# YuxinxinChen/dlrm-yx

Hardware: AMD Instinct MI355X
Metric: DLRM samples/sec fwd+bwd at 1/2/4/8 MI355X; embedding HBM GB/s vs peak (higher is better)
Workload: dtype fp32; 1 GPU; mlperf_terabyte_synthetic; global_batch=2048, local_batch=2048, tables=26, rows_total=54063992, emb_dim=128, lookups_per_bag=1, optimizer=sgd, parallelism=table-sharded emb x1 + dp1, hip_graph=True, capture=whole, bot_sched=auto, tbe_role=True, bottom_parts=0, head_role=True, early_sort=True, feature_pad=False

## Files before the change

dlrm-yx_amd/csrc/gemm.hip:

```cpp
#include <cstdlib>
#include <cstring>
#include <type_traits>

#include "common.hpp"
#include "tbe_bwd_roles.hpp"

#ifndef DLRM_GEMM_STAMP
#define DLRM_GEMM_STAMP(slot)
#endif

namespace {

using f32x16 = __attribute__((ext_vector_type(16))) float;
using f32x4 = __attribute__((ext_vector_type(4))) float;
constexpr int kThreads = 256;
constexpr int kMaxSplit = 32;
constexpr int kMaxGroup = 6;
constexpr int64_t kTicketCap = 16384;
constexpr int kBK = 32;
constexpr int kRasterRows = 4;

struct GemmParams {
  int64_t M, N, K;
  float alpha;
  const float* A;
  int64_t lda;
  const float* B;
  int64_t ldb;
  float* C;
  int64_t ldc;
  int epi;
  const float* bias;
  const float* aux;
  int64_t ldaux;
  int64_t ones_col;
  int layout;
  int tiles_m, tiles_n;
  int splits;
  int block0;
  int64_t kchunk;
  float* ws;
  int* counters;
  int mode;
  float* part;
  const float* alpha_dev;
};

struct GemmGroup {
  GemmParams p[kMaxGroup];
  int n;
  int total;
};

__device__ __forceinline__ int swz_kc(int r) {
  return ((r >> 1) & 7) ^ (((unsigned)((r & 15) - 4) < 8u) ? 2 : 0);
}

template <int MN, int BKT, bool KC, bool VEC, int NT, bool SWZ = false>
struct Stage {
  static_assert(!SWZ || (BKT % 32 == 0 && MN >= 32), "swizzled images: BKT 32 U, MN >= 32");
  static constexpr int PITCH = SWZ ? (KC ? 32 : MN) : (KC ? BKT + 4 : MN + 4);
  static constexpr int SIZE = SWZ ? MN * BKT : (KC ? MN * PITCH : BKT * PITCH);
  __device__ __forceinline__ static int at(int mn, int k) {
    if constexpr (!SWZ) return KC ? mn * PITCH + k : k * PITCH + mn;
    else if constexpr (KC)
      return ((k >> 5) * MN + mn) * 32 + 4 * (((k & 31) >> 2) ^ swz_kc(mn)) + (k & 3);
    else return k * PITCH + (mn ^ (((k >> 3) & 1) << 4));
  }
  static constexpr int NV = MN * BKT / 4 / NT;
  static_assert(NV >= 1 && MN * BKT % (4 * NT) == 0, "panel / thread mismatch");
  float4 regs[NV];

  __device__ __forceinline__ void coords(int q, int& mn, int& k) const {
    if constexpr (KC && SWZ) {
      const int u = q / (MN * 8), r = q - u * (MN * 8);
      mn = r >> 3;
      k = 32 * u + 4 * (r & 7);
    } else if constexpr (KC) {
      mn = q / (BKT / 4);
      k = 4 * (q % (BKT / 4));
    } else {
      k = q / (MN / 4);
      mn = 4 * (q % (MN / 4));
    }
  }

  __device__ __forceinline__ void load(const float* __restrict__ X, int64_t ld, int64_t mn0,
                                       int64_t mnlim, int64_t k0, int64_t klim, int tid) {
    if (VEC && mn0 + MN <= mnlim && k0 + BKT <= klim) {
#pragma unroll
      for (int v = 0; v < NV; ++v) {
        int mn, k;
        coords(tid + v * NT, mn, k);
        const float* ptr = KC ? X + (mn0 + mn) * ld + k0 + k : X + (k0 + k) * ld + mn0 + mn;
        regs[v] = *reinterpret_cast<const float4*>(ptr);
      }
      return;
    }
#pragma unroll
    for (int v = 0; v < NV; ++v) {
      int mn, k;
      coords(tid + v * NT, mn, k);
      const int64_t gmn = mn0 + mn, gk = k0 + k;
      const float* ptr = KC ? X + gmn * ld + gk : X + gk * ld + gmn;
      const bool full = KC ? (gmn < mnlim && gk + 3 < klim) : (gk < klim && gmn + 3 < mnlim);
      if (VEC && full) {
        regs[v] = *reinterpret_cast<const float4*>(ptr);
      } else {
        float e[4];
#pragma unroll
        for (int c = 0; c < 4; ++c) {
          const bool ok = KC ? (gmn < mnlim && gk + c < klim) : (gk < klim && gmn + c < mnlim);
          e[c] = ok ? ptr[c] : 0.f;
        }
        regs[v] = make_float4(e[0], e[1], e[2], e[3]);
      }
    }
  }

  __device__ __forceinline__ void load_one(int v, const float* __restrict__ X, int64_t ld,
                                           int64_t mn0, int64_t mnlim, int64_t k0, int64_t klim,
                                           int tid, bool fast) {
    int mn, k;
    coords(tid + v * NT, mn, k);
    const int64_t gmn = mn0 + mn, gk = k0 + k;
    const float* ptr = KC ? X + gmn * ld + gk : X + gk * ld + gmn;
    if (VEC && fast) {
      regs[v] = *reinterpret_cast<const float4*>(ptr);
      return;
    }
    float e[4];
#pragma unroll
    for (int c = 0; c < 4; ++c) {
      const bool ok = KC ? (gmn < mnlim && gk + c < klim) : (gk < klim && gmn + c < mnlim);
      e[c] = ok ? ptr[c] : 0.f;
    }
    regs[v] = make_float4(e[0], e[1], e[2], e[3]);
  }

  __device__ __forceinline__ void load_one4(int v, __amdgpu_buffer_rsrc_t rsrc, int64_t ld,
                                            int64_t mn0, int64_t mnlim, int64_t k0, int64_t klim,
                                            int tid) {
    int mn, k;
    coords(tid + v * NT, mn, k);
    const int64_t gmn = mn0 + mn, gk = k0 + k;
    const bool ok = gmn < mnlim && gk < klim;
    const int64_t e = KC ? gmn * ld + gk : gk * ld + gmn;
    const int off = ok ? (int)(e * 4) : 0x7ffffff0;
    const auto t = __builtin_amdgcn_raw_buffer_load_b128(rsrc, off, 0, 0);
    regs[v] = __builtin_bit_cast(float4, t);
  }

  struct Fetch {
    int off[NV];
    int kpos[NV];
  };
  __device__ __forceinline__ void fetch_init(Fetch& f, int64_t ld, int64_t mn0, int64_t mnlim,
                                             int64_t kbeg, int tid) const {
#pragma unroll
    for (int v = 0; v < NV; ++v) {
      int mn, k;
      coords(tid + v * NT, mn, k);
      const int64_t gmn = mn0 + mn, gk = kbeg + k;
      const int64_t e = KC ? gmn * ld + gk : gk * ld + gmn;
      f.off[v] = (KC || gmn < mnlim) ? (int)(e * 4) : -1;
      f.kpos[v] = k;
    }
  }
  __device__ __forceinline__ void fetch4(int v, const Fetch& f, __amdgpu_buffer_rsrc_t rsrc,
                                         int tile_step, int t, int kt0, int klim) {
    const bool ok = f.off[v] >= 0 && kt0 + f.kpos[v] < klim;
    const int off = ok ? f.off[v] + t * tile_step : 0x7ffffff0;
    regs[v] = __builtin_bit_cast(float4, __builtin_amdgcn_raw_buffer_load_b128(rsrc, off, 0, 0));
  }

  __device__ __forceinline__ void fetch4s(int v, const Fetch& f, __amdgpu_buffer_rsrc_t rsrc,
                                          int soff) {
    const int off = f.off[v] >= 0 ? f.off[v] : 0x7ffffff0;
    regs[v] = __builtin_bit_cast(float4, __builtin_amdgcn_raw_buffer_load_b128(rsrc, off, soff, 0));
  }

  __device__ __forceinline__ void store_one(int v, float* __restrict__ lds, int tid) const {
    int mn, k;
    coords(tid + v * NT, mn, k);
    *reinterpret_cast<float4*>(lds + at(mn, k)) = regs[v];
  }

  __device__ __forceinline__ void store(float* __restrict__ lds, int tid) const {
#pragma unroll
    for (int v = 0; v < NV; ++v) store_one(v, lds, tid);
  }

  template <int NS>
  __device__ __forceinline__ void frag(const float* __restrict__ lds, int off, int l32, int kbase,
                                       float (&f)[NS]) const {
    static_assert(NS % 4 == 0, "fragment length");
    if constexpr (KC) {
#pragma unroll
      for (int c = 0; c < NS / 4; ++c) {
        const float4 v = *reinterpret_cast<const float4*>(lds + at(off + l32, kbase + 4 * c));
        f[4 * c + 0] = v.x;
        f[4 * c + 1] = v.y;
        f[4 * c + 2] = v.z;
        f[4 * c + 3] = v.w;
      }
    } else {
#pragma unroll
      for (int s = 0; s < NS; ++s) f[s] = lds[at(off + l32, kbase + s)];
    }
  }
};

__device__ __forceinline__ float add_f32(float a, float b) {
// ... 158 lines not shown
                                            rr, (o + tid * NV + 4 * q) * 4, 0, 16));
#pragma unroll
    for (int i = 0; i < FM; ++i)
      tr[i] = __builtin_bit_cast(float, __builtin_amdgcn_raw_buffer_load_b32(
                                            rr, (o + BM * BN + rrow + i * rs_stride) * 4, 0, 16));
  };
  auto add_rec = [&](const float4 (&t)[NV / 4], const float (&tr)[FM], bool first) {
#pragma unroll
    for (int q = 0; q < NV / 4; ++q) {
      v[4 * q + 0] = first ? t[q].x : v[4 * q + 0] + t[q].x;
      v[4 * q + 1] = first ? t[q].y : v[4 * q + 1] + t[q].y;
      v[4 * q + 2] = first ? t[q].z : v[4 * q + 2] + t[q].z;
      v[4 * q + 3] = first ? t[q].w : v[4 * q + 3] + t[q].w;
    }
#pragma unroll
    for (int i = 0; i < FM; ++i) rs[i] = first ? tr[i] : rs[i] + tr[i];
  };
  int s = 0;
  for (; s + 1 < p.splits; s += 2) {
    float4 t0[NV / 4], t1[NV / 4];
    float r0[FM], r1[FM];
    load_rec(s, t0, r0);
    load_rec(s + 1, t1, r1);
    add_rec(t0, r0, s == 0);
    add_rec(t1, r1, false);
  }
  if (s < p.splits) {
    float4 t0[NV / 4];
    float r0[FM];
    load_rec(s, t0, r0);
    add_rec(t0, r0, s == 0);
  }
  return true;
}

template <int BM, int BN, int WGM, int WGN, bool RS, int FM, int FN>
__device__ __forceinline__ void finish_tile(const GemmParams& p, float alpha,
                                            const f32x4 (&acc)[FM][FN], float (&rs)[FM], int tile,
                                            int split, int tn, int64_t m0, int64_t n0,
                                            float* smem) {
  constexpr int WM = BM / WGM, WN = BN / WGN;
  const int tid = threadIdx.x;
  const int wave = tid >> 6;
  const int lane = tid & 63;
  const int kq = lane >> 4;
  const int l16 = lane & 15;
  const int wm0 = (wave / WGN) * WM;
  const int wn0 = (wave % WGN) * WN;
  const bool rs_owner = RS && tn == 0 && (wave % WGN) == 0 && kq == 0;

  constexpr int NV = FM * FN * 4;
  float v[NV];
#pragma unroll
  for (int i = 0; i < FM; ++i)
#pragma unroll
    for (int j = 0; j < FN; ++j)
#pragma unroll
      for (int r = 0; r < 4; ++r) v[(i * FN + j) * 4 + r] = acc[i][j][r];
  if (p.mode == DLRM_GEMM_PARTIAL) {
    float* slab = p.part + (int64_t)split * p.M * p.N;
    if (p.M * p.N * 4 < 0x7ff00000LL) {
      const __amdgpu_buffer_rsrc_t rp = __builtin_amdgcn_make_buffer_rsrc(
          (void*)slab, (short)0, (int)(p.M * p.N * 4), 0x00020000);
#pragma unroll
      for (int i = 0; i < FM; ++i)
#pragma unroll
        for (int j = 0; j < FN; ++j) {
          const int col = (int)(n0 + wn0 + j * 16 + l16);
#pragma unroll
          for (int r = 0; r < 4; ++r) {
            const int row = (int)(m0 + wm0 + i * 16 + 4 * kq + r);
            buf_st(v[(i * FN + j) * 4 + r], rp,
                   row < p.M && col < p.N ? (int)(((int64_t)row * p.N + col) * 4) : kOob);
          }
        }
    } else {
#pragma unroll
      for (int i = 0; i < FM; ++i)
#pragma unroll
        for (int j = 0; j < FN; ++j) {
          const int64_t col = n0 + wn0 + j * 16 + l16;
#pragma unroll
          for (int r = 0; r < 4; ++r) {
            const int64_t row = m0 + wm0 + i * 16 + 4 * kq + r;
            if (row < p.M && col < p.N) slab[row * p.N + col] = v[(i * FN + j) * 4 + r];
          }
        }
    }
    if (rs_owner) {
      float* rslab = p.part + (int64_t)p.splits * p.M * p.N + (int64_t)split * p.M;
#pragma unroll
      for (int i = 0; i < FM; ++i) {
        const int64_t row = m0 + wm0 + i * 16 + l16;
        if (row < p.M) rslab[row] = rs[i];
      }
    }
    return;
  }
  if (!splitk_reduce<BM, BN, NV, FM>(p, tile, split, v, rs, wm0 + l16, 16, rs_owner, smem))
    return;
  if (epi_fits(p)) {
    int row[NV], col[NV];
    bool ok[NV];
    float w[NV];
#pragma unroll
    for (int i = 0; i < FM; ++i)
#pragma unroll
      for (int j = 0; j < FN; ++j)
#pragma unroll
        for (int r = 0; r < 4; ++r) {
          const int q = (i * FN + j) * 4 + r;
          row[q] = (int)(m0 + wm0 + i * 16 + 4 * kq + r);
          col[q] = (int)(n0 + wn0 + j * 16 + l16);
          ok[q] = col[q] < p.N;
          w[q] = dlrm_scale(alpha, v[q]);
        }
    store_elems_any<NV>(p, row, col, ok, w);
    if constexpr (RS) {
      int rrow[FM], rcol[FM];
      bool rok[FM];
      float rw[FM];
#pragma unroll
      for (int i = 0; i < FM; ++i) {
        rrow[i] = (int)(m0 + wm0 + i * 16 + l16);
        rcol[i] = (int)p.ones_col;
        rok[i] = rs_owner;
        rw[i] = dlrm_scale(alpha, rs[i]);
      }
      store_elems_any<FM>(p, rrow, rcol, rok, rw);
    }
    return;
  }
#pragma unroll
  for (int i = 0; i < FM; ++i)
#pragma unroll
    for (int j = 0; j < FN; ++j) {
      const int64_t col = n0 + wn0 + j * 16 + l16;
#pragma unroll
      for (int r = 0; r < 4; ++r) {
        const int64_t row = m0 + wm0 + i * 16 + 4 * kq + r;
        if (row < p.M && col < p.N) store_epilogue(p, row, col, alpha, v[(i * FN + j) * 4 + r]);
      }
    }
  if (rs_owner) {
#pragma unroll
    for (int i = 0; i < FM; ++i) {
      const int64_t row = m0 + wm0 + i * 16 + l16;
      if (row < p.M) store_epilogue(p, row, p.ones_col, alpha, rs[i]);
    }
  }
}


template <int BM, int BN, int WGM, int WGN, bool A_KC, bool B_KC, bool RS, int U = 1>
__device__ __forceinline__ void pipe_body(const GemmParams& p, int lb, float* smem) {
  static_assert(U == 1 || U % 2 == 0, "sub-tiles per stage: 1 or even");
  constexpr int NT = WGM * WGN * 64;
  constexpr int WM = BM / WGM, WN = BN / WGN;
  constexpr int FM = WM / 16, FN = WN / 16;
  static_assert(FM >= 1 && FN >= 1, "wave sub-tile");
  constexpr int KL = kBK / 4;
  constexpr int BKT = kBK * U;
  using SA = Stage<BM, BKT, A_KC, true, NT, true>;
  using SB = Stage<BN, BKT, B_KC, true, NT, true>;
  constexpr int NS = SA::NV + SB::NV;
  static_assert(NS <= U * KL - 1, "staging must finish before the barrier step");

  const float alpha = dlrm_resolve_lr(p.alpha_dev, p.alpha);
  const int tile = lb / p.splits;
  const int split = lb - tile * p.splits;
  int tm, tn;
  {
    constexpr int G = kRasterRows;
    const int per_group = G * p.tiles_n;
    const int grp = tile / per_group, first = grp * G;
    const int gsz = p.tiles_m - first < G ? p.tiles_m - first : G;
    const int pos = tile - grp * per_group;
    tm = first + pos % gsz;
    tn = pos / gsz;
  }
  if constexpr (RS) {
    if (tn != 0) return pipe_body<BM, BN, WGM, WGN, A_KC, B_KC, false, U>(p, lb, smem);
  }
  const int64_t m0 = (int64_t)tm * BM;
  const int64_t n0 = (int64_t)tn * BN;
  const int64_t kbeg = (int64_t)split * p.kchunk;
  const int64_t kend = (kbeg + p.kchunk < p.K) ? kbeg + p.kchunk : p.K;

  const int tid = threadIdx.x;
  const int wave = tid >> 6;
  const int lane = tid & 63;
  const int kq = lane >> 4;
  const int l16 = lane & 15;
  const int wm0 = (wave / WGN) * WM;
  const int wn0 = (wave % WGN) * WN;

  f32x4 acc[FM][FN];
#pragma unroll
  for (int i = 0; i < FM; ++i)
#pragma unroll
    for (int j = 0; j < FN; ++j) acc[i][j] = f32x4{0.f, 0.f, 0.f, 0.f};
  float rs[FM];
#pragma unroll
  for (int i = 0; i < FM; ++i) rs[i] = 0.f;

  const int nsub = (int)((kend - kbeg + kBK - 1) / kBK);
  const int nk = (nsub + U - 1) / U;
  SA sa;
  SB sb;
  const int64_t a_ext = A_KC ? (p.M - 1) * p.lda + p.K : (p.K - 1) * p.lda + p.M;
  const int64_t b_ext = B_KC ? (p.N - 1) * p.ldb + p.K : (p.K - 1) * p.ldb + p.N;
  const __amdgpu_buffer_rsrc_t ra =
      __builtin_amdgcn_make_buffer_rsrc((void*)p.A, (short)0, (int)(a_ext * 4), 0x00020000);
  const __amdgpu_buffer_rsrc_t rb =
      __builtin_amdgcn_make_buffer_rsrc((void*)p.B, (short)0, (int)(b_ext * 4), 0x00020000);
  typename SA::Fetch fa;
  typename SB::Fetch fb;
  sa.fetch_init(fa, p.lda, m0, p.M, kbeg, tid);
  sb.fetch_init(fb, p.ldb, n0, p.N, kbeg, tid);
  const int a_step = A_KC ? BKT * 4 : (int)(BKT * p.lda * 4);
  const int b_step = B_KC ? BKT * 4 : (int)(BKT * p.ldb * 4);
  const int kb32 = (int)kbeg, kend32 = (int)kend;
  auto fetch_one = [&](int c, int t) {
    if (c < SA::NV)
      sa.fetch4(c, fa, ra, a_step, t, kb32 + t * BKT, kend32);
    else
      sb.fetch4(c - SA::NV, fb, rb, b_step, t, kb32 + t * BKT, kend32);
  };
  auto fetch_any = [&](int c, int t, auto fast) {
    if constexpr (decltype(fast)::value) {
      if (c < SA::NV)
        sa.fetch4s(c, fa, ra, t * a_step);
      else
        sb.fetch4s(c - SA::NV, fb, rb, t * b_step);
    } else {
      fetch_one(c, t);
    }
  };
  auto put_one = [&](int c, float* buf) {
    if (c < SA::NV)
      sa.store_one(c, buf, tid);
    else
      sb.store_one(c - SA::NV, buf + SA::SIZE, tid);
  };
  auto read_frags = [&](const float* buf, int u, float (&a)[FM][KL], float (&b)[FN][KL]) {
#pragma unroll
    for (int i = 0; i < FM; ++i)
      sa.template frag<KL>(buf, wm0 + i * 16, l16, u * kBK + kq * KL, a[i]);
#pragma unroll
    for (int j = 0; j < FN; ++j)
      sb.template frag<KL>(buf + SA::SIZE, wn0 + j * 16, l16, u * kBK + kq * KL, b[j]);
  };
  auto mfma_step = [&](float (&ca)[FM][KL], float (&cb)[FN][KL], int s) {
#pragma unroll
    for (int i = 0; i < FM; ++i)
#pragma unroll
      for (int j = 0; j < FN; ++j)
        acc[i][j] = __builtin_amdgcn_mfma_f32_16x16x4f32(ca[i][s], cb[j][s], acc[i][j], 0, 0, 0);
    if constexpr (RS) {
#pragma unroll
      for (int i = 0; i < FM; ++i) rs[i] = add_f32(rs[i], ca[i][s]);
    }
  };

  float a[FM][KL], b[FN][KL];
  DLRM_GEMM_STAMP(0);
  {
    SA sa1;
    SB sb1;
#pragma unroll
    for (int c = 0; c < NS; ++c) fetch_one(c, 0);
#pragma unroll
    for (int c = 0; c < SA::NV; ++c) sa1.fetch4(c, fa, ra, a_step, 1, kb32 + BKT, kend32);
#pragma unroll
    for (int c = 0; c < SB::NV; ++c) sb1.fetch4(c, fb, rb, b_step, 1, kb32 + BKT, kend32);
#pragma unroll
    for (int c = 0; c < NS; ++c) put_one(c, smem);
#pragma unroll
    for (int c = 0; c < SA::NV; ++c) sa.regs[c] = sa1.regs[c];
#pragma unroll
    for (int c = 0; c < SB::NV; ++c) sb.regs[c] = sb1.regs[c];
  }
  __syncthreads();
  read_frags(smem, 0, a, b);
  DLRM_GEMM_STAMP(1);

  auto subtile = [&](int kt, int u, float (&ca)[FM][KL], float (&cb)[FN][KL],
                     float (&na)[FM][KL], float (&nb)[FN][KL], auto fast) {
    const float* cur = smem + (kt & 1) * (SA::SIZE + SB::SIZE);
    float* nbuf = smem + ((kt + 1) & 1) * (SA::SIZE + SB::SIZE);
    const bool last = u == U - 1;
    if (!last) read_frags(cur, u + 1, na, nb);
#pragma unroll
    for (int s = 0; s < KL - 1; ++s) {
      mfma_step(ca, cb, s);
      const int g = u * KL + s;
      if (g < NS) {
        put_one(g, nbuf);
        fetch_any(g, kt + 2, fast);
      }
      __builtin_amdgcn_sched_barrier(0);
    }
    if (!last) {
      mfma_step(ca, cb, KL - 1);
      const int g = u * KL + KL - 1;
      if (g < NS) {
        put_one(g, nbuf);
        fetch_any(g, kt + 2, fast);
      }
      __builtin_amdgcn_sched_barrier(0);
    } else {
      __syncthreads();
      read_frags(nbuf, 0, na, nb);
      __builtin_amdgcn_sched_barrier(0);
      mfma_step(ca, cb, KL - 1);
    }
  };
  float a1[FM][KL], b1[FN][KL];
  if constexpr (U == 1) {
    const std::true_type fast{};
    const std::false_type slow{};
    for (int kt = 0; kt < nk; kt += 2) {
      if (kb32 + (kt + 3) * BKT <= kend32)
        subtile(kt, 0, a, b, a1, b1, fast);
      else
        subtile(kt, 0, a, b, a1, b1, slow);
      DLRM_GEMM_STAMP(2 + kt);
      if (kt + 1 >= nk) break;
      if (kb32 + (kt + 4) * BKT <= kend32)
        subtile(kt + 1, 0, a1, b1, a, b, fast);
      else
        subtile(kt + 1, 0, a1, b1, a, b, slow);
      DLRM_GEMM_STAMP(3 + kt);
    }
  } else {
    for (int kt = 0; kt < nk; ++kt) {
#pragma unroll
      for (int u = 0; u < U; u += 2) {
        subtile(kt, u, a, b, a1, b1, std::false_type{});
        subtile(kt, u + 1, a1, b1, a, b, std::false_type{});
      }
    }
  }

#pragma unroll
  for (int i = 0; i < FM; ++i) {
    rs[i] += __shfl_xor(rs[i], 16, 64);
    rs[i] += __shfl_xor(rs[i], 32, 64);
  }
  DLRM_GEMM_STAMP(-2);
  finish_tile<BM, BN, WGM, WGN, RS>(p, alpha, acc, rs, tile, split, tn, m0, n0, smem);
  DLRM_GEMM_STAMP(-1);
}

__device__ __forceinline__ void reduce_body(const GemmParams& p, int lb) {
  const float alpha = dlrm_resolve_lr(p.alpha_dev, p.alpha);
  const int64_t MN = p.M * p.N;
  const int64_t i = (int64_t)lb * blockDim.x + threadIdx.x;
  const int64_t n4 = MN / 4;
  const int S = p.splits;
  if (i < n4) {
    const float4* src = reinterpret_cast<const float4*>(p.part) + i;
    const int64_t stride = MN / 4;
    float4 acc = src[0];
    for (int s0 = 1; s0 < S; s0 += 8) {
      float4 t[8];
#pragma unroll
      for (int u = 0; u < 8; ++u)
        if (s0 + u < S) t[u] = src[(int64_t)(s0 + u) * stride];
#pragma unroll
      for (int u = 0; u < 8; ++u)
        if (s0 + u < S) {
          acc.x += t[u].x;
          acc.y += t[u].y;
          acc.z += t[u].z;
          acc.w += t[u].w;
        }
    }
    const int64_t e = 4 * i, row = e / p.N, col = e - row * p.N;
    const float a4[4] = {acc.x, acc.y, acc.z, acc.w};
    store_epilogue<4>(p, row, col, alpha, a4);
  } else if (p.ones_col >= 0 && i - n4 < p.M) {
    const int64_t row = i - n4;
    const float* rsrc = p.part + (int64_t)S * MN + row;
    float acc = rsrc[0];
    for (int s = 1; s < S; ++s) acc += rsrc[(int64_t)s * p.M];
    store_epilogue(p, row, p.ones_col, alpha, acc);
  }
}

template <int BM, int BN, int U = 1>
constexpr int group_smem_floats() {
  return 2 * (BM + BN) * kBK * U;
}

__host__ __device__ constexpr int kind_bit(int layout, bool rs) { return 1 << (rs ? 4 : layout); }

template <int BM, int BN, int WGM, int WGN, int KINDS, int U = 1>
__device__ __forceinline__ void group_body(const GemmGroup& g, int b, float* smem) {
  int q = 0;
#pragma unroll
  for (int i = 1; i < kMaxGroup; ++i)
    if (i < g.n && b >= g.p[i].block0) q = i;
  const GemmParams& p = g.p[q];
  const int nq = (q + 1 < g.n ? g.p[q + 1].block0 : g.total) - p.block0;
  const int lb = xcd_remap(b - p.block0, nq);
  if (p.mode == DLRM_GEMM_REDUCE) return reduce_body(p, lb);
  const int kind = (p.layout == 2 && p.ones_col >= 0) ? 4 : p.layout;
  if constexpr ((KINDS & 1) != 0)
    if (kind == 0) return pipe_body<BM, BN, WGM, WGN, true, true, false, U>(p, lb, smem);
  if constexpr ((KINDS & 2) != 0)
    if (kind == 1) return pipe_body<BM, BN, WGM, WGN, true, false, false, U>(p, lb, smem);
  if constexpr ((KINDS & 4) != 0)
    if (kind == 2) return pipe_body<BM, BN, WGM, WGN, false, false, false, U>(p, lb, smem);
  if constexpr ((KINDS & 8) != 0)
    if (kind == 3) return pipe_body<BM, BN, WGM, WGN, false, true, false, U>(p, lb, smem);
  if constexpr ((KINDS & 16) != 0)
    if (kind == 4) return pipe_body<BM, BN, WGM, WGN, false, false, true, U>(p, lb, smem);
}

template <int BM, int BN, int WGM, int WGN, int KINDS, int U = 1>
__global__ __launch_bounds__(WGM * WGN * 64, 2) void gemm_group_kernel(
    const GemmGroup g) {
  __shared__ __attribute__((aligned(16))) float smem[group_smem_floats<BM, BN, U>()];
  group_body<BM, BN, WGM, WGN, KINDS, U>(g, blockIdx.x, smem);
}

template <int BM, int BN, int WGM, int WGN, int PHASE>
__global__ __launch_bounds__(WGM * WGN * 64, 4) void gemm_role_kernel(const GemmGroup g,
                                                                      const LaunchRole r) {
  __shared__ __attribute__((aligned(16))) float smem[group_smem_floats<BM, BN>()];
  const int b = blockIdx.x;
  if (b < r.blocks) return tbe_role_run<PHASE>(r, b, smem);
  group_body<BM, BN, WGM, WGN, 31>(g, b - r.blocks, smem);
}

template <bool A_KC, bool B_KC>
__global__ __launch_bounds__(kThreads, 2) void gemm_generic_kernel(const GemmParams p) {
  constexpr int BM = 64, BN = 64, BKT = 32;
  constexpr int WM = BM / 2, WN = BN / 2;
  constexpr int NSTEP = BKT / 2;
  using SA = Stage<BM, BKT, A_KC, false, kThreads>;
  using SB = Stage<BN, BKT, B_KC, false, kThreads>;
  __shared__ __attribute__((aligned(16))) float smem[2 * (SA::SIZE + SB::SIZE)];
  float* As0 = smem;
  float* Bs0 = smem + SA::SIZE;
  float* As1 = smem + SA::SIZE + SB::SIZE;
  float* Bs1 = As1 + SA::SIZE;
  const float alpha = dlrm_resolve_lr(p.alpha_dev, p.alpha);
  const int tile = xcd_remap(blockIdx.x, p.tiles_m * p.tiles_n);
  const int tm = tile / p.tiles_n, tn = tile - (tile / p.tiles_n) * p.tiles_n;
  const int64_t m0 = (int64_t)tm * BM, n0 = (int64_t)tn * BN;
  const int tid = threadIdx.x, wave = tid >> 6, lane = tid & 63;
  const int h = lane >> 5, l32 = lane & 31;
  const int wm0 = (wave >> 1) * WM, wn0 = (wave & 1) * WN;
  f32x16 acc, acc2;
#pragma unroll
  for (int r = 0; r < 16; ++r) acc[r] = acc2[r] = 0.f;
  SA sa;
  SB sb;
  const int64_t nk = (p.K + BKT - 1) / BKT;
  if (nk > 0) {
    sa.load(p.A, p.lda, m0, p.M, 0, p.K, tid);
    sb.load(p.B, p.ldb, n0, p.N, 0, p.K, tid);
    sa.store(As0, tid);
    sb.store(Bs0, tid);
  }
  __syncthreads();
  for (int64_t kt = 0; kt < nk; ++kt) {
    const bool odd = kt & 1;
    const float* As = odd ? As1 : As0;
    const float* Bs = odd ? Bs1 : Bs0;
    const bool more = kt + 1 < nk;
    if (more) {
      sa.load(p.A, p.lda, m0, p.M, (kt + 1) * BKT, p.K, tid);
      sb.load(p.B, p.ldb, n0, p.N, (kt + 1) * BKT, p.K, tid);
    }
    float a[NSTEP], b[NSTEP];
    sa.template frag<NSTEP>(As, wm0, l32, h * NSTEP, a);
    sb.template frag<NSTEP>(Bs, wn0, l32, h * NSTEP, b);
#pragma unroll
    for (int s = 0; s < NSTEP; ++s) {
      if (s & 1)
        acc2 = __builtin_amdgcn_mfma_f32_32x32x2f32(a[s], b[s], acc2, 0, 0, 0);
      else
        acc = __builtin_amdgcn_mfma_f32_32x32x2f32(a[s], b[s], acc, 0, 0, 0);
    }
    if (more) {
      sa.store(odd ? As0 : As1, tid);
      sb.store(odd ? Bs0 : Bs1, tid);
    }
    __syncthreads();
  }
  acc += acc2;
  const int64_t col = n0 + wn0 + l32;
#pragma unroll
  for (int r = 0; r < 16; ++r) {
    const int64_t row = m0 + wm0 + (r & 3) + 8 * (r >> 2) + 4 * h;
    if (row < p.M && col < p.N) store_epilogue(p, row, col, alpha, acc[r]);
  }
}

__global__ __launch_bounds__(kThreads) void gemm_rowsum_kernel(const GemmParams p, bool a_kc) {
  __shared__ float part[4][64];
  const float alpha = dlrm_resolve_lr(p.alpha_dev, p.alpha);
  const int tid = threadIdx.x, r = tid & 63, ks = tid >> 6;
  const int64_t m = (int64_t)blockIdx.x * 64 + r;
  float s = 0.f;
  if (m < p.M)
    for (int64_t k = ks; k < p.K; k += 4) s += a_kc ? p.A[m * p.lda + k] : p.A[k * p.lda + m];
  part[ks][r] = s;
  __syncthreads();
  if (ks == 0 && m < p.M)
    store_epilogue(p, m, p.ones_col, alpha, ((part[0][r] + part[1][r]) + part[2][r]) + part[3][r]);
}

struct Plan {
  int splits = 1;
  int64_t kchunk = 0;
};

Plan make_plan(int64_t s, int64_t K) {
  if (s > kMaxSplit) s = kMaxSplit;
  int64_t smax = dlrm::ceil_div(K, kBK);
  if (s > smax) s = smax;
  if (s < 1) s = 1;
  int64_t kchunk = dlrm::ceil_div(dlrm::ceil_div(K, s), kBK) * kBK;
  if (kchunk < kBK) kchunk = kBK;
  Plan pl;
  pl.splits = (int)dlrm::ceil_div(K, kchunk);
  pl.kchunk = kchunk;
  return pl;
}

struct Desc {
  int32_t trans_a, trans_b;
  int64_t M, N, K;
  float alpha;
  const float *A, *B;
  int64_t lda, ldb;
  float* C;
  int64_t ldc;
  int32_t epi;
  const float* bias;
  const float* aux;
  int64_t ldaux;
  int64_t ones_col;
  int32_t mode = DLRM_GEMM_FULL;
  int32_t splits = 0;
  float* part = nullptr;
  const float* alpha_dev = nullptr;
};

inline bool aligned16(const void* p) { return (reinterpret_cast<uintptr_t>(p) & 15) == 0; }

bool pipe_ok(const Desc& d) {
  const bool a_kc = !d.trans_a, b_kc = d.trans_b != 0;
  const int64_t a_ext = a_kc ? (d.M - 1) * d.lda + d.K : (d.K - 1) * d.lda + d.M;
  const int64_t b_ext = b_kc ? (d.N - 1) * d.ldb + d.K : (d.K - 1) * d.ldb + d.N;
  return aligned16(d.A) && aligned16(d.B) && d.lda % 4 == 0 && d.ldb % 4 == 0 && d.K % 4 == 0 &&
         (a_kc || d.M % 4 == 0) && (b_kc || d.N % 4 == 0) && a_ext * 4 < 0x7ff00000LL &&
         b_ext * 4 < 0x7ff00000LL;
}

int layout_of(const Desc& d) {
  const bool a_kc = !d.trans_a, b_kc = d.trans_b != 0;
  return a_kc ? (b_kc ? 0 : 1) : (b_kc ? 3 : 2);
}

struct PlanEntry {
  int64_t M, N, K;
  int layout, bm, bn, split;
  int wm = 2, wn = 2;
};

constexpr PlanEntry kPlans[] = {
#include "gemm_plans.inc"
    {0, 0, 0, 0, 64, 64, 1},
};

bool tile_ok(int bm, int bn, int wm, int wn) {
  return wm == 2 && wn == 2 &&
         ((bm == 64 && bn == 64) || (bm == 128 && bn == 64) || (bm == 64 && bn == 128) ||
          (bm == 32 && bn == 64) || (bm == 64 && bn == 32) || (bm == 32 && bn == 32));
}

struct Tile {
  int bm = 64, bn = 32, wm = 2, wn = 2;
  bool operator==(const Tile& o) const {
    return bm == o.bm && bn == o.bn && wm == o.wm && wn == o.wn;
  }
};

void plan_one(const Desc& d, Tile& t, Plan& pl) {
  t = Tile{64, 64, 2, 2};
  if (d.mode == DLRM_GEMM_REDUCE) {
    pl.splits = d.splits;
    pl.kchunk = 0;
    return;
  }
  if (d.mode == DLRM_GEMM_PARTIAL && d.splits > 0) {
    Desc q = d;
    q.mode = DLRM_GEMM_FULL;
    plan_one(q, t, pl);
    pl = make_plan(d.splits, d.K);
    return;
  }
  if (const int64_t tile = dlrm::tuning(DLRM_TUNE_GEMM_TILE)) {
    const int a = (int)(tile / 1000), b = (int)(tile % 1000);
    if (tile_ok(a, b, 2, 2)) t = Tile{a, b, 2, 2};
    const int64_t fs = dlrm::tuning(DLRM_TUNE_GEMM_SPLIT);
    pl = make_plan(fs > 0 ? fs : 1, d.K);
    return;
  }
  const bool use_table = true;
  if (use_table)
    for (const PlanEntry& e : kPlans)
      if (e.M == d.M && e.N == d.N && e.K == d.K && e.layout == layout_of(d)) {
        t = Tile{e.bm, e.bn, e.wm, e.wn};
        pl = make_plan(e.split, d.K);
        return;
      }
  t = Tile{64, 32, 2, 2};
  const int64_t tiles = dlrm::ceil_div(d.M, 64) * dlrm::ceil_div(d.N, 32);
  const int target = d.mode == DLRM_GEMM_PARTIAL ? 512 : 256;
  int64_t s = 1;
  while (tiles * s < target && dlrm::ceil_div(d.K, s + 1) >= 256 && s < kMaxSplit) ++s;
  pl = make_plan(s, d.K);
}

void plan_launch(int n, const Desc* d, Tile& t, Plan* pl) {
  bool first = true;
  t = Tile{64, 64, 2, 2};
  for (int i = 0; i < n; ++i) {
    Tile a;
    plan_one(d[i], a, pl[i]);
    if (d[i].mode == DLRM_GEMM_REDUCE) continue;
    if (first) {
      t = a;
      first = false;
    } else if (!(a == t)) {
      t = Tile{64, 32, 2, 2};
    }
  }
  if (t.bm == 128 && t.bn == 128) t = Tile{64, 32, 2, 2};
}

int64_t split_tiles(int n, const Desc* d, const Tile& t, const Plan* pl) {
  int64_t tick = 0;
  for (int i = 0; i < n; ++i)
    if (pl[i].splits > 1 && d[i].mode == DLRM_GEMM_FULL)
      tick += dlrm::ceil_div(d[i].M, t.bm) * dlrm::ceil_div(d[i].N, t.bn);
  return tick;
}

size_t group_ws_bytes(int n, const Desc* d, const Tile& t, const Plan* pl) {
  const int bm = t.bm, bn = t.bn;
  WsCarver c(nullptr);
  c.take<int>(kTicketCap);
  bool any = false;
  for (int i = 0; i < n; ++i)
    if (pl[i].splits > 1 && d[i].mode == DLRM_GEMM_FULL) {
      any = true;
      const int64_t tiles = dlrm::ceil_div(d[i].M, bm) * dlrm::ceil_div(d[i].N, bn);
      c.take<float>((size_t)tiles * pl[i].splits * (bm * bn + bm));
    }
  return any ? c.used + 256 : 0;
}

template <int BM, int BN, int U = 1, int WGM = 2, int WGN = 2>
int launch_group(int n, const Desc* d, const Plan* pl, void* ws, size_t ws_bytes,
                 const LaunchRole* role, int phase, hipStream_t st) {
  constexpr int NT = WGM * WGN * 64;
  GemmGroup g{};
  g.n = n;
  WsCarver c(ws);
  int* tickets = c.take<int>(kTicketCap);
  int64_t tick = 0, blocks = 0;
  for (int i = 0; i < n; ++i) {
    GemmParams& p = g.p[i];
    p.M = d[i].M, p.N = d[i].N, p.K = d[i].K, p.alpha = d[i].alpha;
    p.A = d[i].A, p.lda = d[i].lda, p.B = d[i].B, p.ldb = d[i].ldb;
    p.C = d[i].C, p.ldc = d[i].ldc, p.epi = d[i].epi, p.bias = d[i].bias;
    p.aux = d[i].aux, p.ldaux = d[i].ldaux, p.ones_col = d[i].ones_col;
    p.layout = layout_of(d[i]);
    p.mode = d[i].mode;
    p.part = d[i].part;
    p.alpha_dev = d[i].alpha_dev;
    p.tiles_m = (int)dlrm::ceil_div(p.M, BM);
    p.tiles_n = (int)dlrm::ceil_div(p.N, BN);
    p.splits = pl[i].splits;
    p.kchunk = pl[i].kchunk > 0 ? pl[i].kchunk : kBK;
    p.block0 = (int)blocks;
    if (p.mode == DLRM_GEMM_REDUCE) {
      blocks += dlrm::ceil_div(p.M * p.N / 4 + (p.ones_col >= 0 ? p.M : 0), NT);
      continue;
    }
    if (p.splits > 1 && p.mode == DLRM_GEMM_FULL) {
      const int64_t tiles = (int64_t)p.tiles_m * p.tiles_n;
      p.counters = tickets + tick;
      p.ws = c.take<float>((size_t)tiles * p.splits * (BM * BN + BM));
      tick += tiles;
    }
    blocks += (int64_t)p.tiles_m * p.tiles_n * p.splits;
  }
  DLRM_REQUIRE(tick <= kTicketCap && blocks < INT32_MAX, DLRM_ERR_UNSUPPORTED,
               "dlrm_gemm_f32: too many split tiles in one launch");
  DLRM_REQUIRE(tick == 0 || (ws && ws_bytes >= c.used), DLRM_ERR_WORKSPACE,
               "dlrm_gemm_f32: workspace too small");
  g.total = (int)blocks;
  int kinds = 0;
  for (int i = 0; i < n; ++i)
    if (g.p[i].mode != DLRM_GEMM_REDUCE)
      kinds |= kind_bit(g.p[i].layout, g.p[i].layout == 2 && g.p[i].ones_col >= 0);
  if constexpr (U == 1 && ((BM == 64 && BN == 32) || (BM == 32 && BN == 64))) {
    if (role) {
      static_assert(NT == 256, "the update passes run 256-thread workgroups");
      DLRM_REQUIRE((int64_t)role->blocks + blocks < INT32_MAX, DLRM_ERR_UNSUPPORTED,
                   "dlrm_gemm_f32_group_role: too many workgroups");
      const dim3 grid(role->blocks + g.total), block(NT);
      if (phase == 1)
        hipLaunchKernelGGL((gemm_role_kernel<BM, BN, WGM, WGN, 1>), grid, block, 0, st, g, *role);
      else if (phase == 2)
        hipLaunchKernelGGL((gemm_role_kernel<BM, BN, WGM, WGN, 2>), grid, block, 0, st, g, *role);
      else
        hipLaunchKernelGGL((gemm_role_kernel<BM, BN, WGM, WGN, 4>), grid, block, 0, st, g, *role);
      DLRM_LAUNCH_CHECK("dlrm_gemm_f32_group_role");
      return DLRM_OK;
    }
  } else {
    DLRM_REQUIRE(!role, DLRM_ERR_UNSUPPORTED, "dlrm_gemm_f32_group_role: tile %dx%d/%d", BM, BN,
                 U);
  }
  const dim3 grid(g.total), block(NT);
  switch (kinds) {
#define K_(M_)                                                                          \
  case M_:                                                                             \
    hipLaunchKernelGGL((gemm_group_kernel<BM, BN, WGM, WGN, M_, U>), grid, block, 0, st, g); \
    break;
    K_(0) K_(1) K_(2) K_(4) K_(8) K_(16) K_(2 | 16) K_(2 | 4) K_(4 | 16)
#undef K_
    default:
      hipLaunchKernelGGL((gemm_group_kernel<BM, BN, WGM, WGN, 31, U>), grid, block, 0, st, g);
  }
  DLRM_LAUNCH_CHECK("dlrm_gemm_f32");
  return DLRM_OK;
}

int launch_generic(const Desc& d, hipStream_t st) {
  GemmParams p{};
  p.M = d.M, p.N = d.N, p.K = d.K, p.alpha = d.alpha;
  p.A = d.A, p.lda = d.lda, p.B = d.B, p.ldb = d.ldb;
  p.C = d.C, p.ldc = d.ldc, p.epi = d.epi, p.bias = d.bias;
  p.aux = d.aux, p.ldaux = d.ldaux, p.ones_col = d.ones_col;
  p.alpha_dev = d.alpha_dev;
  p.tiles_m = (int)dlrm::ceil_div(p.M, 64);
  p.tiles_n = (int)dlrm::ceil_div(p.N, 64);
  p.splits = 1;
  const bool a_kc = !d.trans_a, b_kc = d.trans_b != 0;
  const dim3 grid(p.tiles_m * p.tiles_n), block(kThreads);
  if (a_kc && b_kc)
    hipLaunchKernelGGL((gemm_generic_kernel<true, true>), grid, block, 0, st, p);
  else if (a_kc)
    hipLaunchKernelGGL((gemm_generic_kernel<true, false>), grid, block, 0, st, p);
  else if (b_kc)
    hipLaunchKernelGGL((gemm_generic_kernel<false, true>), grid, block, 0, st, p);
  else
    hipLaunchKernelGGL((gemm_generic_kernel<false, false>), grid, block, 0, st, p);
  DLRM_LAUNCH_CHECK("dlrm_gemm_f32 (generic)");
  if (d.ones_col >= 0) {
    hipLaunchKernelGGL(gemm_rowsum_kernel, dim3(dlrm::ceil_div(d.M, 64)), dim3(kThreads), 0, st, p,
                       a_kc);
    DLRM_LAUNCH_CHECK("dlrm_gemm_f32 (row sum)");
  }
  return DLRM_OK;
}

int check_desc(const Desc& d) {
  DLRM_ARG(d.mode >= DLRM_GEMM_FULL && d.mode <= DLRM_GEMM_REDUCE, "dlrm_gemm_f32: bad mode");
  if (d.mode != DLRM_GEMM_FULL) {
    DLRM_ARG(d.part, "dlrm_gemm_f32: PARTIAL/REDUCE need a partial buffer");
    DLRM_ARG(d.mode != DLRM_GEMM_REDUCE || (d.splits >= 1 && d.N % 4 == 0 && d.M >= 0 && d.C &&
                                            d.ldc >= d.N),
             "dlrm_gemm_f32: REDUCE needs splits >= 1, N %% 4 == 0 and C");
    if (d.mode == DLRM_GEMM_REDUCE) {
      DLRM_ARG(d.ones_col < 0 || (d.ones_col >= d.N && d.ones_col < d.ldc),
               "dlrm_gemm_f32: ones_col outside [N, ldc)");
      return DLRM_OK;
    }
    DLRM_REQUIRE(pipe_ok(d), DLRM_ERR_UNSUPPORTED,
                 "dlrm_gemm_f32: PARTIAL needs 16-B aligned operands, K %% 4 == 0");
    DLRM_ARG(d.splits <= 0 || make_plan(d.splits, d.K).splits == d.splits,
             "dlrm_gemm_f32: PARTIAL splits=%d is not a normalized count for K=%lld "
             "(use dlrm_gemm_f32_splits)", (int)d.splits, (long long)d.K);
  }
  DLRM_ARG(d.M >= 0 && d.N >= 0 && d.K >= 0, "dlrm_gemm_f32: negative size");
  if (d.M == 0 || (d.N == 0 && d.ones_col < 0)) return DLRM_OK;
  DLRM_ARG(d.C, "dlrm_gemm_f32: null C");
  DLRM_ARG(d.K == 0 || (d.A && d.B), "dlrm_gemm_f32: null A/B");
  DLRM_ARG(d.epi >= DLRM_EPI_STORE && d.epi <= DLRM_EPI_RELU, "dlrm_gemm_f32: bad epilogue");
  DLRM_ARG(!(d.epi == DLRM_EPI_BIAS || d.epi == DLRM_EPI_BIAS_RELU) || d.bias,
           "dlrm_gemm_f32: epilogue needs bias");
  DLRM_ARG(d.epi != DLRM_EPI_DRELU || (d.aux && d.ldaux >= d.N), "dlrm_gemm_f32: DRELU needs aux");
  DLRM_ARG(d.ldc >= d.N && (d.ones_col < 0 || (d.ones_col >= d.N && d.ones_col < d.ldc)),
           "dlrm_gemm_f32: ldc < N or ones_col outside [N, ldc)");
  DLRM_ARG(d.trans_a ? d.lda >= d.M : d.lda >= d.K, "dlrm_gemm_f32: bad lda");
  DLRM_ARG(d.trans_b ? d.ldb >= d.K : d.ldb >= d.N, "dlrm_gemm_f32: bad ldb");
  DLRM_REQUIRE(dlrm::ceil_div(d.M, 64) * dlrm::ceil_div(d.N, 64) < (int64_t)INT32_MAX / kMaxSplit,
               DLRM_ERR_UNSUPPORTED, "dlrm_gemm_f32: too large");
  return DLRM_OK;
}

size_t ws_for(int n, const Desc* d) {
  Desc q[kMaxGroup];
  int m = 0;
  for (int i = 0; i < n; ++i)
    if (d[i].M > 0 && d[i].N > 0 && d[i].K > 0 && pipe_ok(d[i])) q[m++] = d[i];
  if (m == 0) return 0;
  Tile t;
  Plan pl[kMaxGroup];
  plan_launch(m, q, t, pl);
  const size_t a = group_ws_bytes(m, q, t, pl);
  const size_t b = group_ws_bytes(m, q, Tile{64, 32, 2, 2}, pl);
  return a > b ? a : b;
}

int run(int n, const Desc* d, void* ws, size_t ws_bytes, hipStream_t st,
        const LaunchRole* role = nullptr, int phase = 0) {
  DLRM_ARG(n >= (role ? 0 : 1) && n <= kMaxGroup, "dlrm_gemm_f32_group: 1..%d problems",
           kMaxGroup);
  Desc q[kMaxGroup];
  int m = 0;
  for (int i = 0; i < n; ++i) {
    const int rc = check_desc(d[i]);
    if (rc != DLRM_OK) return rc;
    if (d[i].M == 0 || (d[i].N == 0 && d[i].ones_col < 0)) continue;
    if (d[i].mode == DLRM_GEMM_REDUCE) {
      q[m++] = d[i];
      continue;
    }
    if (d[i].K == 0 || !pipe_ok(d[i])) {
      const int r2 = launch_generic(d[i], st);
      if (r2 != DLRM_OK) return r2;
      continue;
    }
    q[m++] = d[i];
  }
  if (m == 0 && !role) return DLRM_OK;
  Tile t;
  Plan pl[kMaxGroup];
  plan_launch(m, q, t, pl);
  if (role && !(t == Tile{64, 32, 2, 2}) && !(t == Tile{32, 64, 2, 2})) {
    if (split_tiles(m, q, Tile{64, 32, 2, 2}, pl) > kTicketCap) {
      const int rc = launch_group<64, 32>(0, q, pl, ws, ws_bytes, role, phase, st);
      if (rc != DLRM_OK) return rc;
      return run(m, q, ws, ws_bytes, st);
    }
    t = Tile{64, 32, 2, 2};
  }
  const size_t need = group_ws_bytes(m, q, t, pl);
  if (need > 0 && (!ws || ws_bytes < need)) {
    for (int i = 0; i < m; ++i)
      if (q[i].mode == DLRM_GEMM_FULL) pl[i] = make_plan(1, q[i].K);
  }
  if (t.bm == 128) return launch_group<128, 64>(m, q, pl, ws, ws_bytes, role, phase, st);
  if (t.bn == 128) return launch_group<64, 128>(m, q, pl, ws, ws_bytes, role, phase, st);
  if (t.bm == 32 && t.bn == 32)
    return launch_group<32, 32>(m, q, pl, ws, ws_bytes, role, phase, st);
  if (t.bm == 32) return launch_group<32, 64>(m, q, pl, ws, ws_bytes, role, phase, st);
  if (t.bn == 32) return launch_group<64, 32>(m, q, pl, ws, ws_bytes, role, phase, st);
  return launch_group<64, 64>(m, q, pl, ws, ws_bytes, role, phase, st);
}

Desc desc_of(const dlrm_gemm_problem& g) {
  Desc d;
  d.trans_a = g.trans_a, d.trans_b = g.trans_b;
  d.M = g.M, d.N = g.N, d.K = g.K, d.alpha = g.alpha;
  d.A = g.A, d.lda = g.lda, d.B = g.B, d.ldb = g.ldb;
  d.C = g.C, d.ldc = g.ldc, d.epi = g.epilogue, d.bias = g.bias;
  d.aux = g.aux, d.ldaux = g.ld_aux, d.ones_col = g.ones_col;
  d.mode = g.mode, d.splits = g.splits, d.part = g.partial;
  d.alpha_dev = g.alpha_dev;
  return d;
}

}

extern "C" size_t dlrm_gemm_f32_workspace_size(int32_t trans_a, int32_t trans_b, int64_t M,
                                               int64_t N, int64_t K) {
  if (M <= 0 || N <= 0 || K <= 0) return 0;
  Desc d{};
  d.trans_a = trans_a, d.trans_b = trans_b, d.M = M, d.N = N, d.K = K;
  d.lda = ((trans_a ? M : K) + 3) / 4 * 4, d.ldb = ((trans_b ? K : N) + 3) / 4 * 4;
  d.A = d.B = reinterpret_cast<const float*>(256);
  d.ones_col = -1;
  return ws_for(1, &d);
// ... 68 lines not shown
```

Measured before the change: 5.379 million samples/s.

## Split k-tile fragment reads into halves and move barrier earlier in GEMM pipeline

Restructures the MFMA main loop so each k-tile's LDS fragments are read in two halves: the second half is loaded while the first half's MFMAs run. The block barrier and the prefetch of the next buffer's first-half fragments now happen at a configurable mid-tile step instead of just before the final MFMA. This hides LDS read latency and barrier stalls behind MFMA work. It also removes the multi-subtile (U) template path, at the cost of more live fragment registers.

```diff
diff --git a/dlrm-yx_amd/csrc/gemm.hip b/dlrm-yx_amd/csrc/gemm.hip
--- a/dlrm-yx_amd/csrc/gemm.hip
+++ b/dlrm-yx_amd/csrc/gemm.hip
@@ -7,6 +7,9 @@
 
 #ifndef DLRM_GEMM_STAMP
 #define DLRM_GEMM_STAMP(slot)
+#endif
+#ifndef DLRM_GEMM_BARRIER_STEP
+#define DLRM_GEMM_BARRIER_STEP 4
 #endif
 
 namespace {
@@ -58,7 +61,7 @@
 
 template <int MN, int BKT, bool KC, bool VEC, int NT, bool SWZ = false>
 struct Stage {
-  static_assert(!SWZ || (BKT % 32 == 0 && MN >= 32), "swizzled images: BKT 32 U, MN >= 32");
+  static_assert(!SWZ || (BKT % 32 == 0 && MN >= 32), "swizzled images: BKT % 32 == 0, MN >= 32");
   static constexpr int PITCH = SWZ ? (KC ? 32 : MN) : (KC ? BKT + 4 : MN + 4);
   static constexpr int SIZE = SWZ ? MN * BKT : (KC ? MN * PITCH : BKT * PITCH);
   __device__ __forceinline__ static int at(int mn, int k) {
@@ -523,19 +526,21 @@
 }
 
 
-template <int BM, int BN, int WGM, int WGN, bool A_KC, bool B_KC, bool RS, int U = 1>
+template <int BM, int BN, int WGM, int WGN, bool A_KC, bool B_KC, bool RS>
 __device__ __forceinline__ void pipe_body(const GemmParams& p, int lb, float* smem) {
-  static_assert(U == 1 || U % 2 == 0, "sub-tiles per stage: 1 or even");
   constexpr int NT = WGM * WGN * 64;
   constexpr int WM = BM / WGM, WN = BN / WGN;
   constexpr int FM = WM / 16, FN = WN / 16;
   static_assert(FM >= 1 && FN >= 1, "wave sub-tile");
   constexpr int KL = kBK / 4;
-  constexpr int BKT = kBK * U;
+  constexpr int KH = KL / 2;
+  constexpr int BKT = kBK;
   using SA = Stage<BM, BKT, A_KC, true, NT, true>;
   using SB = Stage<BN, BKT, B_KC, true, NT, true>;
   constexpr int NS = SA::NV + SB::NV;
-  static_assert(NS <= U * KL - 1, "staging must finish before the barrier step");
+  constexpr int BAR = DLRM_GEMM_BARRIER_STEP > NS - 1 ? DLRM_GEMM_BARRIER_STEP : NS - 1;
+  static_assert(DLRM_GEMM_BARRIER_STEP >= KH && BAR <= KL - 2,
+                "barrier after H1 is read (k-step >= 4), one k-step left to cover H0");
 
   const float alpha = dlrm_resolve_lr(p.alpha_dev, p.alpha);
   const int tile = lb / p.splits;
@@ -551,7 +556,7 @@
     tn = pos / gsz;
   }
   if constexpr (RS) {
-    if (tn != 0) return pipe_body<BM, BN, WGM, WGN, A_KC, B_KC, false, U>(p, lb, smem);
+    if (tn != 0) return pipe_body<BM, BN, WGM, WGN, A_KC, B_KC, false>(p, lb, smem);
   }
   const int64_t m0 = (int64_t)tm * BM;
   const int64_t n0 = (int64_t)tn * BN;
@@ -575,8 +580,7 @@
 #pragma unroll
   for (int i = 0; i < FM; ++i) rs[i] = 0.f;
 
-  const int nsub = (int)((kend - kbeg + kBK - 1) / kBK);
-  const int nk = (nsub + U - 1) / U;
+  const int nk = (int)((kend - kbeg + kBK - 1) / kBK);
   SA sa;
   SB sb;
   const int64_t a_ext = A_KC ? (p.M - 1) * p.lda + p.K : (p.K - 1) * p.lda + p.M;
@@ -614,15 +618,17 @@
     else
       sb.store_one(c - SA::NV, buf + SA::SIZE, tid);
   };
-  auto read_frags = [&](const float* buf, int u, float (&a)[FM][KL], float (&b)[FN][KL]) {
+  auto read_a = [&](const float* buf, int h, float (&a)[FM][KH]) {
 #pragma unroll
     for (int i = 0; i < FM; ++i)
-      sa.template frag<KL>(buf, wm0 + i * 16, l16, u * kBK + kq * KL, a[i]);
+      sa.template frag<KH>(buf, wm0 + i * 16, l16, kq * KL + h * KH, a[i]);
+  };
+  auto read_b = [&](const float* buf, int h, float (&b)[FN][KH]) {
 #pragma unroll
     for (int j = 0; j < FN; ++j)
-      sb.template frag<KL>(buf + SA::SIZE, wn0 + j * 16, l16, u * kBK + kq * KL, b[j]);
+      sb.template frag<KH>(buf + SA::SIZE, wn0 + j * 16, l16, kq * KL + h * KH, b[j]);
   };
-  auto mfma_step = [&](float (&ca)[FM][KL], float (&cb)[FN][KL], int s) {
+  auto mfma_step = [&](float (&ca)[FM][KH], float (&cb)[FN][KH], int s) {
 #pragma unroll
     for (int i = 0; i < FM; ++i)
 #pragma unroll
@@ -634,7 +640,7 @@
     }
   };
 
-  float a[FM][KL], b[FN][KL];
+  float a[FM][KH], b[FN][KH];
   DLRM_GEMM_STAMP(0);
   {
     SA sa1;
@@ -653,64 +659,52 @@
     for (int c = 0; c < SB::NV; ++c) sb.regs[c] = sb1.regs[c];
   }
   __syncthreads();
-  read_frags(smem, 0, a, b);
+  read_a(smem, 0, a);
+  read_b(smem, 0, b);
   DLRM_GEMM_STAMP(1);
 
-  auto subtile = [&](int kt, int u, float (&ca)[FM][KL], float (&cb)[FN][KL],
-                     float (&na)[FM][KL], float (&nb)[FN][KL], auto fast) {
+  float ha[FM][KH], hb[FN][KH];
+  auto ktile = [&](int kt, float (&ca)[FM][KH], float (&cb)[FN][KH], float (&na)[FM][KH],
+                   float (&nb)[FN][KH], auto fast) {
     const float* cur = smem + (kt & 1) * (SA::SIZE + SB::SIZE);
     float* nbuf = smem + ((kt + 1) & 1) * (SA::SIZE + SB::SIZE);
-    const bool last = u == U - 1;
-    if (!last) read_frags(cur, u + 1, na, nb);
-#pragma unroll
-    for (int s = 0; s < KL - 1; ++s) {
-      mfma_step(ca, cb, s);
-      const int g = u * KL + s;
-      if (g < NS) {
-        put_one(g, nbuf);
-        fetch_any(g, kt + 2, fast);
+#pragma unroll
+    for (int s = 0; s < KL; ++s) {
+      if (s == 0) read_a(cur, 1, ha);
+      if (s == 1) read_b(cur, 1, hb);
+      if (s < KH)
+        mfma_step(ca, cb, s);
+      else
+        mfma_step(ha, hb, s - KH);
+      if (s < NS) {
+        put_one(s, nbuf);
+        fetch_any(s, kt + 2, fast);
       }
       __builtin_amdgcn_sched_barrier(0);
-    }
-    if (!last) {
-      mfma_step(ca, cb, KL - 1);
-      const int g = u * KL + KL - 1;
-      if (g < NS) {
-        put_one(g, nbuf);
-        fetch_any(g, kt + 2, fast);
+      if (s == BAR) {
+        __syncthreads();
+        read_a(nbuf, 0, na);
+        read_b(nbuf, 0, nb);
+        __builtin_amdgcn_sched_barrier(0);
       }
-      __builtin_amdgcn_sched_barrier(0);
-    } else {
-      __syncthreads();
-      read_frags(nbuf, 0, na, nb);
-      __builtin_amdgcn_sched_barrier(0);
-      mfma_step(ca, cb, KL - 1);
     }
   };
-  float a1[FM][KL], b1[FN][KL];
-  if constexpr (U == 1) {
+  float a1[FM][KH], b1[FN][KH];
+  {
     const std::true_type fast{};
     const std::false_type slow{};
     for (int kt = 0; kt < nk; kt += 2) {
       if (kb32 + (kt + 3) * BKT <= kend32)
-        subtile(kt, 0, a, b, a1, b1, fast);
+        ktile(kt, a, b, a1, b1, fast);
       else
-        subtile(kt, 0, a, b, a1, b1, slow);
+        ktile(kt, a, b, a1, b1, slow);
       DLRM_GEMM_STAMP(2 + kt);
       if (kt + 1 >= nk) break;
       if (kb32 + (kt + 4) * BKT <= kend32)
-        subtile(kt + 1, 0, a1, b1, a, b, fast);
+        ktile(kt + 1, a1, b1, a, b, fast);
       else
-        subtile(kt + 1, 0, a1, b1, a, b, slow);
+        ktile(kt + 1, a1, b1, a, b, slow);
       DLRM_GEMM_STAMP(3 + kt);
-    }
-  } else {
-    for (int kt = 0; kt < nk; ++kt) {
-#pragma unroll
-      for (int u = 0; u < U; u += 2) {
-        subtile(kt, u, a, b, a1, b1, std::false_type{});
-        subtile(kt, u + 1, a1, b1, a, b, std::false_type{});
-      }
     }
   }
 
@@ -760,14 +754,14 @@
   }
 }
 
-template <int BM, int BN, int U = 1>
+template <int BM, int BN>
 constexpr int group_smem_floats() {
-  return 2 * (BM + BN) * kBK * U;
+  return 2 * (BM + BN) * kBK;
 }
 
 __host__ __device__ constexpr int kind_bit(int layout, bool rs) { return 1 << (rs ? 4 : layout); }
 
-template <int BM, int BN, int WGM, int WGN, int KINDS, int U = 1>
+template <int BM, int BN, int WGM, int WGN, int KINDS>
 __device__ __forceinline__ void group_body(const GemmGroup& g, int b, float* smem) {
   int q = 0;
 #pragma unroll
@@ -779,22 +773,22 @@
   if (p.mode == DLRM_GEMM_REDUCE) return reduce_body(p, lb);
   const int kind = (p.layout == 2 && p.ones_col >= 0) ? 4 : p.layout;
   if constexpr ((KINDS & 1) != 0)
-    if (kind == 0) return pipe_body<BM, BN, WGM, WGN, true, true, false, U>(p, lb, smem);
+    if (kind == 0) return pipe_body<BM, BN, WGM, WGN, true, true, false>(p, lb, smem);
   if constexpr ((KINDS & 2) != 0)
-    if (kind == 1) return pipe_body<BM, BN, WGM, WGN, true, false, false, U>(p, lb, smem);
+    if (kind == 1) return pipe_body<BM, BN, WGM, WGN, true, false, false>(p, lb, smem);
   if constexpr ((KINDS & 4) != 0)
-    if (kind == 2) return pipe_body<BM, BN, WGM, WGN, false, false, false, U>(p, lb, smem);
+    if (kind == 2) return pipe_body<BM, BN, WGM, WGN, false, false, false>(p, lb, smem);
   if constexpr ((KINDS & 8) != 0)
-    if (kind == 3) return pipe_body<BM, BN, WGM, WGN, false, true, false, U>(p, lb, smem);
+    if (kind == 3) return pipe_body<BM, BN, WGM, WGN, false, true, false>(p, lb, smem);
   if constexpr ((KINDS & 16) != 0)
-    if (kind == 4) return pipe_body<BM, BN, WGM, WGN, false, false, true, U>(p, lb, smem);
-}
-
-template <int BM, int BN, int WGM, int WGN, int KINDS, int U = 1>
+    if (kind == 4) return pipe_body<BM, BN, WGM, WGN, false, false, true>(p, lb, smem);
+}
+
+template <int BM, int BN, int WGM, int WGN, int KINDS>
 __global__ __launch_bounds__(WGM * WGN * 64, 2) void gemm_group_kernel(
     const GemmGroup g) {
-  __shared__ __attribute__((aligned(16))) float smem[group_smem_floats<BM, BN, U>()];
-  group_body<BM, BN, WGM, WGN, KINDS, U>(g, blockIdx.x, smem);
+  __shared__ __attribute__((aligned(16))) float smem[group_smem_floats<BM, BN>()];
+  group_body<BM, BN, WGM, WGN, KINDS>(g, blockIdx.x, smem);
 }
 
 template <int BM, int BN, int WGM, int WGN, int PHASE>
@@ -1039,7 +1033,7 @@
   return any ? c.used + 256 : 0;
 }
 
-template <int BM, int BN, int U = 1, int WGM = 2, int WGN = 2>
+template <int BM, int BN, int WGM = 2, int WGN = 2>
 int launch_group(int n, const Desc* d, const Plan* pl, void* ws, size_t ws_bytes,
                  const LaunchRole* role, int phase, hipStream_t st) {
   constexpr int NT = WGM * WGN * 64;
@@ -1084,7 +1078,7 @@
   for (int i = 0; i < n; ++i)
     if (g.p[i].mode != DLRM_GEMM_REDUCE)
       kinds |= kind_bit(g.p[i].layout, g.p[i].layout == 2 && g.p[i].ones_col >= 0);
-  if constexpr (U == 1 && ((BM == 64 && BN == 32) || (BM == 32 && BN == 64))) {
+  if constexpr ((BM == 64 && BN == 32) || (BM == 32 && BN == 64)) {
     if (role) {
       static_assert(NT == 256, "the update passes run 256-thread workgroups");
       DLRM_REQUIRE((int64_t)role->blocks + blocks < INT32_MAX, DLRM_ERR_UNSUPPORTED,
@@ -1100,19 +1094,18 @@
       return DLRM_OK;
     }
   } else {
-    DLRM_REQUIRE(!role, DLRM_ERR_UNSUPPORTED, "dlrm_gemm_f32_group_role: tile %dx%d/%d", BM, BN,
-                 U);
+    DLRM_REQUIRE(!role, DLRM_ERR_UNSUPPORTED, "dlrm_gemm_f32_group_role: tile %dx%d", BM, BN);
   }
   const dim3 grid(g.total), block(NT);
   switch (kinds) {
 #define K_(M_)                                                                          \
   case M_:                                                                             \
-    hipLaunchKernelGGL((gemm_group_kernel<BM, BN, WGM, WGN, M_, U>), grid, block, 0, st, g); \
+    hipLaunchKernelGGL((gemm_group_kernel<BM, BN, WGM, WGN, M_>), grid, block, 0, st, g); \
     break;
     K_(0) K_(1) K_(2) K_(4) K_(8) K_(16) K_(2 | 16) K_(2 | 4) K_(4 | 16)
 #undef K_
     default:
-      hipLaunchKernelGGL((gemm_group_kernel<BM, BN, WGM, WGN, 31, U>), grid, block, 0, st, g);
+      hipLaunchKernelGGL((gemm_group_kernel<BM, BN, WGM, WGN, 31>), grid, block, 0, st, g);
   }
   DLRM_LAUNCH_CHECK("dlrm_gemm_f32");
   return DLRM_OK;
```

Result: no change. 5.432 million samples/s, median of 6 (+1.0%).
